# OminiX-ai/OminiX-MLX

Hardware: AMD Instinct MI355X
Metric: decode_tokens_per_sec (higher is better)
Workload: dtype bf16

## Files before the change

include/omx.h:

```cpp
#ifndef OMX_H
#define OMX_H

#include <stddef.h>
#include <stdint.h>

#ifdef __cplusplus
extern "C" {
#endif

typedef enum omx_dtype_ {
    OMX_BOOL = 0, OMX_UINT8 = 1, OMX_UINT16 = 2, OMX_UINT32 = 3, OMX_UINT64 = 4,
    OMX_INT8 = 5, OMX_INT16 = 6, OMX_INT32 = 7, OMX_INT64 = 8,
    OMX_FLOAT16 = 9, OMX_FLOAT32 = 10, OMX_FLOAT64 = 11, OMX_BFLOAT16 = 12, OMX_COMPLEX64 = 13
} omx_dtype;

typedef void* omx_stream;

const char* omx_version(void);
int omx_experiments_built(void);
typedef void (*omx_error_handler_func)(const char* msg, void* data);
void omx_set_error_handler(omx_error_handler_func handler, void* data, void (*dtor)(void*));
const char* omx_last_error(void);
void omx_clear_error(void);
int omx_device_count(int* count);
// ... 119 lines not shown
int omx_qwen3_batch_create_kv(omx_qwen3_batch* out, omx_qwen3 m, int n_slots, int max_context, int kv_bits);
int omx_qwen3_batch_kv_bytes(omx_qwen3_batch b, size_t* bytes);
int omx_qwen3_batch_kv_read(omx_qwen3_batch b, int slot, int layer, int first, int n, void* k_rows, void* v_rows, void* k_scales,
                            void* k_biases, void* v_scales, void* v_biases);
int omx_qwen3_batch_debug_attention(omx_qwen3_batch b, int layer, const int* slots, int n, const void* q, void* out);
int omx_qwen3_batch_destroy(omx_qwen3_batch b);
int omx_qwen3_batch_set_sampler(omx_qwen3_batch b, int slot, float temperature, uint64_t seed);
int omx_qwen3_batch_set_sampling(omx_qwen3_batch b, int slot, const omx_sampling* p, uint64_t seed);
int omx_qwen3_batch_prefill(omx_qwen3_batch b, int slot, const uint32_t* prompt, int n_prompt, uint32_t* first_token);
int omx_qwen3_batch_decode(omx_qwen3_batch b, const int* slots, int n_slots, int n_steps, uint32_t* tokens_out);
int omx_qwen3_batch_logits(omx_qwen3_batch b, int slot, void* host_bf16, int n);
int omx_qwen3_batch_offset(omx_qwen3_batch b, int slot, int* offset);
int omx_qwen3_batch_trim(omx_qwen3_batch b, int slot, int n, uint32_t next_token);
int omx_qwen3_batch_reset(omx_qwen3_batch b, int slot);
int omx_qwen3_batch_fork(omx_qwen3_batch b, int src, int dst, int resample, uint32_t* first_token);
int omx_qwen3_batch_shared(omx_qwen3_batch b, int slot, int* owner, int* shared_len);
int omx_qwen3_batch_last_decode_ms(omx_qwen3_batch b, float* ms);
int omx_bench_qwen3_per_op(omx_qwen3 model, const omx_qwen3_config* cfg, const uint32_t* prompt, int n_prompt, int n_new,
                           uint32_t* tokens_out, double* prefill_ms, double* ms_per_token, double* calls_per_token);
int omx_qwen3_last_decode_ms(omx_qwen3 m, float* ms);
int omx_qwen3_last_prefill_ms(omx_qwen3 m, float* ms);
int omx_qwen3_dequant_bytes(omx_qwen3 m, size_t* bytes);
int omx_qwen3_debug_read(omx_qwen3 m, const char* name, void* host, size_t n_elems);
int omx_debug_gemv(void* out, unsigned long long* argmax_slot, const void* x, const void* norm_w, const void* resid, const void* bias,
                   const void* w0, const void* w1, const void* w2, int n0, int n1, int N, int K, int pro, int epi, int f16, float eps,
                   int single_round, omx_stream stream);
int omx_debug_gemv_grid(int N, int K);
typedef struct omx_gemv_ex_ {
    void* out; unsigned long long* argmax_slot; int argmax_slot_n;
    const void* x; const void* norm_w; const void* resid; const void* bias;
    const void* w0; const void* w1; const void* w2; int n0, n1, N, K, pro, epi, f16; float eps; int single_round;
    int rows_per_wave, row_offset;
    const float* x_partial; int x_partial_n; void* x_out; const void* out_scale;
    int n_batch, x_div; long long x_bstride, out_bstride_bytes; const unsigned* w_sel; long long w_estride; int w_sel_lo, w_sel_n;
    int dry_run;
    int route_nv, route_ksplit, route_tail, route_rows_per_wave, route_blocks;
} omx_gemv_ex;
int omx_debug_gemv_ex(omx_gemv_ex* a, omx_stream stream);
typedef struct omx_qgemv_member_ { const void* w; const void* scales; const void* biases; int n, bits, group; } omx_qgemv_member;
typedef struct omx_qgemv_ex_ {
    omx_qgemv_member m[3];
    int N, K, group, bits, pro, epi; float eps; int single_round;
    int scales_f16, use_sb, use_tiles, mfma, row_offset, rolled_stage;
    int n_batch, x_div; const unsigned* w_sel; long long w_estride, s_estride; int w_sel_lo, w_sel_n, n_experts;
    const void* x; const void* norm_w; const void* resid;
    void* out; float* out_f32; unsigned long long* argmax_slot; int argmax_slot_n;
// ... 226 lines not shown
```

ominix-mlx_amd/csrc/attn.hpp:

```cpp
#pragma once
#include "common.hpp"

namespace omx {

struct AttnDecodeArgs {
    const bf16_t* q;
    const bf16_t* k;
    const bf16_t* v;
    int64_t kv_batch_stride, kv_head_stride;
    int B, H, Hkv, Tk;
    float scale;
    int mask_mode;
    const void* mask;
    int nsplit;
    float* ws_o;
    float* ws_ml;
    bf16_t* out;
    int64_t q_bs, q_hs;
    int causal_tail;
};

struct AttnStepArgs {
    const bf16_t* qkv;
    bf16_t* k;
    bf16_t* v;
    int64_t kv_head_stride;
    int H, Hkv, cap;
    float scale, eps;
    const bf16_t* q_norm_w;
    const bf16_t* k_norm_w;
    const float* rope_cur;
    const int* pos_ptr;
    const unsigned* seq_ptr;
    unsigned tag_mul, tag_add;
    int chunk;
    int nsplit;
    uint64_t* ws;
    bf16_t* out;
    unsigned* abort_flag;
    unsigned long long* trace;
    const bf16_t* o_w;
    const bf16_t* o_resid;
    bf16_t* o_out;
    float* o_out_f32;
// ... 28 lines not shown
```

ominix-mlx_amd/csrc/attn_step.hip:

```cpp
#include <algorithm>

#include "attn.hpp"
#include "act16.hpp"
#include "gemv_parts.hpp"
#include "granule.hpp"
#include "launch_timing.hpp"

namespace omx {

namespace {

constexpr int kBlock = 512;
constexpr int kWaves = 8;
constexpr unsigned kSpinLimit = 1u << 15;

template <int N>
__device__ __forceinline__ float swap_halves(float v) {
    if (N == 16) return dpp_f<0x128>(v);
    return dpp_f<0x1B>(dpp_f<kDppHalfMirror>(v));
}

template <bool F16 = false>
__device__ __forceinline__ void unpack8(const u32x4 r, float (&x)[8]) {
#pragma unroll
// ... 79 lines not shown
}

constexpr int kKU = 3;

template <bool F16>
__device__ __forceinline__ float dot8_16(const u32x4 a, const u32x4 b) {
    if constexpr (!F16) return dot8_bf16(a, b);
    float d = 0.f;
#pragma unroll
    for (int e = 0; e < 4; ++e) d = Act16<true>::dot2(a[e], b[e], d);
    return d;
}

__device__ __forceinline__ float dot8_chain(const u32x4 w, const u32x4 xp, float acc) {
#pragma unroll
    for (int i = 0; i < 4; ++i) {
        acc = fmaf(bf16lo(w[i]), bf16lo(xp[i]), acc);
        acc = fmaf(bf16hi(w[i]), bf16hi(xp[i]), acc);
    }
    return acc;
}

constexpr int kORows = 4;

template <int NVW>
__device__ __forceinline__ void oproj_await_vector(const AttnStepArgs& a, u32x4* sm_x, unsigned tag, int lane, int wave) {
    asm volatile("s_waitcnt vmcnt(0)" ::: "memory");
    if (wave == 0) {
        constexpr int SEGS = NVW * 8;
        const uint64_t* probe = a.xg + (size_t)min(lane, SEGS - 1) * 32 + 31;
        for (unsigned spins = 0; spins < kSpinLimit; ++spins) {
            const unsigned long long g = ld_granule(probe);
            if (__all((unsigned)(g >> 32) == tag)) break;
            __builtin_amdgcn_s_sleep(4);
        }
    }
    __syncthreads();
    constexpr int GP = (NVW + 1) / 2;
    static_assert((NVW * 256) % GP == 0, "a thread takes all of its granules or none");
    bool done = (int)threadIdx.x * GP >= NVW * 256;
    unsigned* sx = reinterpret_cast<unsigned*>(sm_x);
    for (unsigned spins = 0;; ++spins) {
        if (!done) {
            unsigned long long g[GP];
#pragma unroll
            for (int i = 0; i < GP; ++i) g[i] = ld_granule(a.xg + (size_t)threadIdx.x * GP + i);
            bool ok = true;
#pragma unroll
            for (int i = 0; i < GP; ++i) ok &= (unsigned)(g[i] >> 32) == tag;
            if (ok) {
#pragma unroll
                for (int i = 0; i < GP; ++i) sx[threadIdx.x * GP + i] = (unsigned)g[i];
                done = true;
            }
        }
        if (__syncthreads_and(done)) break;
        if (spins >= kSpinLimit) {
            if (threadIdx.x == 0) __hip_atomic_store(a.abort_flag, 1u, __ATOMIC_RELAXED, __HIP_MEMORY_SCOPE_AGENT);
            break;
        }
        __builtin_amdgcn_s_sleep(2);
    }
}

constexpr int kGuPairs = 6, kGuHidden = 4096, kGuNV = kGuHidden / 512;

__device__ __forceinline__ void gateup_issue(const AttnStepArgs& a, u32x4 (*w)[kGuNV], int pair, int lane) {
    const u32x4* g = reinterpret_cast<const u32x4*>(a.gu_gate + (size_t)pair * kGuHidden);
    const u32x4* u = reinterpret_cast<const u32x4*>(a.gu_up + (size_t)pair * kGuHidden);
#pragma unroll
    for (int j = 0; j < kGuNV; ++j) {
        w[0][j] = ld_nt(g + j * 64 + lane);
        w[1][j] = ld_nt(u + j * 64 + lane);
    }
    __builtin_amdgcn_sched_barrier(0);
}

__device__ __forceinline__ void gateup_reduce(const AttnStepArgs& a, const u32x4 (*w)[kGuNV], const u32x4* xs, int pair, int lane) {
    typedef Act16<false> A;
    float acc[2] = {0.f, 0.f};
#pragma unroll
    for (int j = 0; j < kGuNV; ++j) {
        const u32x4 xp = xs[j * 64 + lane];
        float xf[8];
#pragma unroll
        for (int q = 0; q < 4; ++q) {
            xf[2 * q] = A::lo(xp[q]);
            xf[2 * q + 1] = A::hi(xp[q]);
        }
#pragma unroll
        for (int r = 0; r < 2; ++r) acc[r] = dot8(w[r][j], xf, acc[r]);
    }
#pragma unroll
    for (int r = 0; r < 2; ++r) acc[r] = wave_sum(acc[r]);
    if (lane == 0) a.gu_out[pair] = epi_bits<EPI_SWIGLU, A>(acc[0], acc[1], (bf16_t)0, 0);
}

template <bool TRACE>
__device__ __forceinline__ void gateup_phase(const AttnStepArgs& a, u32x4* xs, float* red, const uint16_t* sm_pub, unsigned tag, int lane,
                                             int wave, int pub_row0, int pub_rows, unsigned long long* tr) {
    typedef Act16<false> A;
    const int pair0 = (((int)blockIdx.y * (int)gridDim.x + (int)blockIdx.x) * kWaves + wave) * kGuPairs;
    u32x4 wA[2][kGuNV];
    constexpr int PV = kGuNV * 64 / 256;
    u32x4 nwv[PV];
#pragma unroll
    for (int i = 0; i < PV; ++i) nwv[i] = *(reinterpret_cast<const u32x4*>(a.gu_norm_w) + (threadIdx.x & 255) + i * 256);
    u32x4 wB[2][kGuNV];
    if (wave != 0) gateup_issue(a, wA, pair0, lane);
    lds_barrier();
    if (wave == 0) {
        if (lane < pub_rows / 2) st_granule_u32(a.hg + pub_row0 / 2 + lane, tag, reinterpret_cast<const unsigned*>(sm_pub)[lane]);
        constexpr int GPL = kGuHidden / 2 / 64;
        for (unsigned spins = 0; spins < kSpinLimit; ++spins) {
            const unsigned long long g = ld_granule(a.hg + (size_t)lane * GPL + (GPL - 1));
            if (__all((unsigned)(g >> 32) == tag)) break;
            __builtin_amdgcn_s_sleep(4);
        }
        unsigned long long g[GPL];
        for (unsigned spins = 0;; ++spins) {
#pragma unroll
            for (int i = 0; i < GPL; ++i) g[i] = ld_granule(a.hg + (size_t)i * 64 + lane);
            bool ok = true;
#pragma unroll
            for (int i = 0; i < GPL; ++i) ok &= (unsigned)(g[i] >> 32) == tag;
            if (__all(ok)) break;
            if (spins >= kSpinLimit) {
                if (lane == 0) __hip_atomic_store(a.abort_flag, 1u, __ATOMIC_RELAXED, __HIP_MEMORY_SCOPE_AGENT);
                break;
            }
            __builtin_amdgcn_s_sleep(4);
        }
        unsigned* sx = reinterpret_cast<unsigned*>(xs);
#pragma unroll
        for (int i = 0; i < GPL; ++i) sx[i * 64 + lane] = (unsigned)g[i];
        if (TRACE && lane == 0 && pub_rows > 0) tr[4] = wall_clock64();
        gateup_issue(a, wA, pair0, lane);
    }
    lds_barrier();
    rmsnorm_in_lds<A, PV>(xs, red, nwv, kGuHidden, a.eps, threadIdx.x < 256);
    static_assert(kGuPairs % 2 == 0, "whole double-buffer rounds");
#pragma unroll
    for (int p = 0; p < kGuPairs; p += 2) {
        gateup_issue(a, wB, pair0 + p + 1, lane);
        gateup_reduce(a, wA, xs, pair0 + p, lane);
        if (TRACE && p == 0 && threadIdx.x == 0) tr[7] = wall_clock64();
        if (p + 2 < kGuPairs) gateup_issue(a, wA, pair0 + p + 2, lane);
        gateup_reduce(a, wB, xs, pair0 + p + 1, lane);
    }
}

template <int NVW, int R, bool GU = false>
__device__ __forceinline__ void oproj_phase(const AttnStepArgs& a, u32x4* sm_x, unsigned tag, int lane, int wave, int o_row0,
                                            unsigned long long* tr, uint16_t* sm_pub = nullptr, int pub_row0 = 0) {
    u32x4 ow[R][NVW];
#pragma unroll
    for (int r = 0; r < R; ++r) {
        const int row = min(o_row0 + r, a.o_rows - 1);
        const u32x4* p = reinterpret_cast<const u32x4*>(a.o_w + (size_t)row * (NVW * 512));
#pragma unroll
        for (int j = 0; j < NVW; ++j) ow[r][j] = __builtin_nontemporal_load(p + j * 64 + lane);
    }
    bf16_t o_res[R];
#pragma unroll
    for (int r = 0; r < R; ++r) o_res[r] = a.o_resid[min(o_row0 + r, a.o_rows - 1)];
    __builtin_amdgcn_sched_barrier(0);
    oproj_await_vector<NVW>(a, sm_x, tag, lane, wave);
    if (tr && threadIdx.x == 0) tr[5] = wall_clock64();
    float acc[R];
#pragma unroll
    for (int r = 0; r < R; ++r) acc[r] = 0.f;
// ... 105 lines not shown
            if (o_row0 + r < a.o_rows) a.o_out[o_row0 + r] = f32_to_bf16(bf16_to_f32(o_res[r]) + round_bf16(acc[r]));
    }
    if (tr && threadIdx.x == 0) tr[6] = wall_clock64();
}


template <int D, int GT, bool TRACE, int NVW, bool F16 = false, bool GU = false>
__global__ __launch_bounds__(kBlock, 1) void attn_step_kernel(const AttnStepArgs a) {
    static_assert(!F16 || NVW == 0, "the O projection rides in the launch for bfloat16 models only");
    static_assert(!GU || (NVW == kGuNV && D == 128), "gate/up follows the bf16 O projection of hidden 4096 only");
    typedef Act16<F16> A16;
    constexpr int LPR = D / 8;
    constexpr int TPW = 64 / LPR;
    constexpr bool QO = NVW >= 100;
    constexpr int NV = QO ? NVW - 100 : NVW;
    constexpr bool OPROJ = NV > 0;
    extern __shared__ __attribute__((aligned(16))) unsigned char smem[];
    float* sm_o = reinterpret_cast<float*>(smem);
    float* sm_m = sm_o + kWaves * TPW * GT * D;
    float* sm_l = sm_m + kWaves * GT;
    u32x4* sm_q = reinterpret_cast<u32x4*>(sm_l + kWaves * GT);
    u32x4* sm_x = sm_q + (GT + 1) * LPR;
    float* sm_xsum = reinterpret_cast<float*>(sm_x + NV * 64);

    const int lane = threadIdx.x & 63;
    const int wave = threadIdx.x >> 6;
    const int c = lane % LPR;
    const int sg = lane / LPR;
    const int kvh = blockIdx.x, split = blockIdx.y;
    const int G = a.H / a.Hkv;
    unsigned long long* tr = TRACE ? a.trace + ((size_t)split * a.Hkv + kvh) * 8 : nullptr;
    if (TRACE && threadIdx.x == 0) tr[0] = wall_clock64();

    bf16_t* Kb = a.k + (size_t)kvh * a.kv_head_stride;
    bf16_t* Vb = a.v + (size_t)kvh * a.kv_head_stride;
    const int t_begin = split * a.chunk;
    const int n_units = a.chunk / TPW;

    const bf16_t* kraw = a.qkv + (size_t)a.H * D + (size_t)kvh * D;
    const bool does_q = wave < GT, does_k = wave == GT % kWaves;
    const bf16_t* my_raw = does_q ? a.qkv + (size_t)(kvh * G + min(wave, G - 1)) * D : kraw;
    const u32x4 raw0 = *reinterpret_cast<const u32x4*>(my_raw + c * 8);
    const u32x4 raw1 = *reinterpret_cast<const u32x4*>(kraw + c * 8);
    const u32x4 vnew = *reinterpret_cast<const u32x4*>(kraw + (size_t)a.Hkv * D + c * 8);
    const int i0 = (c % (LPR / 2)) * 8;
    const f32x4* cp = reinterpret_cast<const f32x4*>(a.rope_cur + i0);
    const f32x4* sp = reinterpret_cast<const f32x4*>(a.rope_cur + D / 2 + i0);
    const f32x4 c0 = cp[0], c1 = cp[1], s0 = sp[0], s1 = sp[1];
    u32x4 wq_raw = {0, 0, 0, 0}, wk_raw = {0, 0, 0, 0};
    if (a.q_norm_w) {
        wq_raw = *reinterpret_cast<const u32x4*>(a.q_norm_w + c * 8);
        wk_raw = *reinterpret_cast<const u32x4*>(a.k_norm_w + c * 8);
    }
    u32x4 kr[kKU], vr[kKU];
    auto issue_kv = [&](int u0) {
// ... 149 lines not shown
            }
            uint64_t* gr = a.ws + ((size_t)(kvh * G + g) * a.nsplit + split) * (D + 2);
            st_granule(gr + d, tag, O);
            if (d == 0) {
                st_granule(gr + D, tag, M);
                st_granule(gr + D + 1, tag, L);
            }
        }
    }
    if (TRACE && threadIdx.x == 0) tr[3] = wall_clock64();

    if (OPROJ && split >= G) {
        const int g = ((split - G) * (int)gridDim.x + kvh) * kWaves + wave;
        const bool hi = g < a.o_nhi;
        const int rows = hi ? a.o_rpw : a.o_rpw - 1;
        const int o_row0 = hi ? g * a.o_rpw : a.o_nhi * a.o_rpw + (g - a.o_nhi) * (a.o_rpw - 1);
        unsigned long long* otr = TRACE ? tr : nullptr;
        if constexpr (GU) {
            auto row0_of = [&](int w) { return w < a.o_nhi ? w * a.o_rpw : a.o_nhi * a.o_rpw + (w - a.o_nhi) * (a.o_rpw - 1); };
            const int pub_row0 = row0_of(g - wave), pub_rows = row0_of(g - wave + kWaves) - pub_row0;
            uint16_t* sm_pub = reinterpret_cast<uint16_t*>(sm_l);
            if (rows == 2) oproj_phase<NV, 2, true>(a, sm_x, tag, lane, wave, o_row0, otr, sm_pub, pub_row0);
            else oproj_phase<NV, 3, true>(a, sm_x, tag, lane, wave, o_row0, otr, sm_pub, pub_row0);
            gateup_phase<TRACE>(a, sm_x, sm_m, sm_pub, tag, lane, wave, pub_row0, pub_rows, otr);
            return;
        } else
        if constexpr (QO) {
            if (rows <= 1) oproj_phase_q4<NV, 1>(a, sm_x, sm_xsum, tag, lane, wave, o_row0, otr);
            else if (rows == 2) oproj_phase_q4<NV, 2>(a, sm_x, sm_xsum, tag, lane, wave, o_row0, otr);
            else if (rows == 3) oproj_phase_q4<NV, 3>(a, sm_x, sm_xsum, tag, lane, wave, o_row0, otr);
            else oproj_phase_q4<NV, 4>(a, sm_x, sm_xsum, tag, lane, wave, o_row0, otr);
        } else {
            if (rows <= 1) oproj_phase<(NV > 0 ? NV : 1), 1>(a, sm_x, tag, lane, wave, o_row0, otr);
            else if (rows == 2) oproj_phase<(NV > 0 ? NV : 1), 2>(a, sm_x, tag, lane, wave, o_row0, otr);
            else if (rows == 3) oproj_phase<(NV > 0 ? NV : 1), 3>(a, sm_x, tag, lane, wave, o_row0, otr);
            else oproj_phase<(NV > 0 ? NV : 1), 4>(a, sm_x, tag, lane, wave, o_row0, otr);
        }
        return;
    }

    if (split < G && wave < D / 64) {
        const int head = kvh * G + split;
        const uint64_t* base = a.ws + (size_t)head * a.nsplit * (D + 2);
        bf16_t* out = a.out + (size_t)head * D;
        const int dim = wave * 64 + lane;
        const int nb = (a.nsplit + 15) / 16;
        uint64_t* xg_head = OPROJ ? a.xg + (size_t)head * (D / 2) : nullptr;
        if (nb <= 1) gather_head<D, 1, F16>(a, base, n_active, tag, lane, dim, out, xg_head);
        else if (nb == 2) gather_head<D, 2, F16>(a, base, n_active, tag, lane, dim, out, xg_head);
        else gather_head<D, 3, F16>(a, base, n_active, tag, lane, dim, out, xg_head);
        if (TRACE && threadIdx.x == 0) tr[4] = wall_clock64();
    }
    if constexpr (GU) {
        lds_barrier();
        gateup_phase<TRACE>(a, sm_x, sm_m, nullptr, tag, lane, wave, 0, 0, TRACE ? tr : nullptr);
    }
}

}

int attn_step_block_tokens(int D) { return 64 / (D / 8); }

constexpr int kMaxSplits = 48;
void attn_step_plan(int tk_max, int Hkv, int G, int D, int* chunk, int* nsplit) {
    const int unit = attn_step_block_tokens(D);
    int target = std::max(1, std::min(kMaxSplits, 256 / std::max(Hkv, 1)));
    if (const char* v = getenv("OMX_ATTN_STEP_SPLITS")) target = std::max(1, std::min(kMaxSplits, atoi(v)));
    int ch = unit * ((tk_max + unit * target - 1) / (unit * target));
    if (ch < unit) ch = unit;
    int ns = (tk_max + ch - 1) / ch;
    if (ns < G) ns = G;
    *chunk = ch;
    *nsplit = ns;
}

size_t attn_step_ws_granules(int H, int D) { return (size_t)H * kMaxSplits * (D + 2); }

static int oproj_rows_per_wave(int H, int Hkv, int nsplit, int o_rows) {
    const int waves = (Hkv * nsplit - H) * kWaves;
    return waves > 0 ? (o_rows + waves - 1) / waves : 1 << 20;
}
bool attn_step_oproj_ok(int H, int Hkv, int D, int nsplit, int o_rows) {
    const int K = H * D, nvw = K / 512;
    return K % 512 == 0 && (nvw == 1 || nvw == 2 || nvw == 4 || nvw == 7 || nvw == 8) && oproj_rows_per_wave(H, Hkv, nsplit, o_rows) <= kORows;
}

bool attn_step_oproj_q4_ok(int H, int Hkv, int D, int nsplit, int o_rows, int group) {
    const int K = H * D;
    return (K == 2048 || K == 4096) && (group == 32 || group == 64 || group == 128) && attn_step_oproj_ok(H, Hkv, D, nsplit, o_rows);
}

bool attn_step_gateup_ok(int H, int Hkv, int D, int nsplit, int o_rows, int gu_rows) {
    const int blocks = Hkv * nsplit, waves = (blocks - H) * kWaves;
    if (D != 128 || H * D != kGuHidden || o_rows != kGuHidden || H / std::max(Hkv, 1) != 4 || blocks != 256) return false;
    if (gu_rows != blocks * kWaves * kGuPairs || !attn_step_oproj_ok(H, Hkv, D, nsplit, o_rows)) return false;
    return oproj_rows_per_wave(H, Hkv, nsplit, o_rows) == 3 && (o_rows - waves * 2) % kWaves == 0;
}

int launch_attn_step(const AttnStepArgs& a_in, int D, hipStream_t s) {
    AttnStepArgs a = a_in;
    const int G = a.H / a.Hkv;
    OMX_REQUIRE(a.H % a.Hkv == 0 && G >= 1 && G <= 8, "decode attention: %d query heads over %d KV heads unsupported (group of at most 8)", a.H, a.Hkv);
    OMX_REQUIRE(a.nsplit >= G && a.nsplit <= kMaxSplits && a.chunk > 0 && a.chunk % attn_step_block_tokens(D) == 0 && a.Hkv * a.nsplit <= 256,
                "decode attention: bad split plan (chunk %d, %d splits, group %d, %d kv heads)", a.chunk, a.nsplit, G, a.Hkv);
    OMX_REQUIRE(a.ws && a.rope_cur && a.pos_ptr && a.seq_ptr && a.abort_flag && a.tag_mul > a.tag_add - 1u && a.tag_add >= 1u,
                "decode attention: missing step state");
    int nvw = 0;
    const bool qo = a.o_wq != nullptr;
    if (qo)
        OMX_REQUIRE(!a.o_w && a.o_sb && a.o_out && !a.o_out_f32 && attn_step_oproj_q4_ok(a.H, a.Hkv, D, a.nsplit, a.o_rows, a.o_group),
                    "decode attention + packed O projection: shape does not qualify (H*D = %d, group %d)", a.H * D, a.o_group);
    if (a.o_w || qo) {
        OMX_REQUIRE(a.o_resid && (a.o_out || a.o_out_f32) && a.xg && attn_step_oproj_ok(a.H, a.Hkv, D, a.nsplit, a.o_rows),
                    "decode attention + O projection: shape does not qualify (H*D = %d, %d rows, %d blocks)", a.H * D, a.o_rows, a.Hkv * a.nsplit);
        nvw = a.H * D / 512;
        a.o_rpw = oproj_rows_per_wave(a.H, a.Hkv, a.nsplit, a.o_rows);
        const int waves = (a.Hkv * a.nsplit - a.H) * kWaves;
        a.o_nhi = a.o_rpw > 1 ? a.o_rows - waves * (a.o_rpw - 1) : waves;
// ... 4 lines not shown
                    "decode attention + gate/up: shape does not qualify (%d blocks, %d O rows, %d pairs)", a.Hkv * a.nsplit, a.o_rows, a.gu_rows);
    const dim3 grid(a.Hkv, a.nsplit), block(kBlock);
    const int gt = G <= 1 ? 1 : G <= 2 ? 2 : G <= 4 ? 4 : 8;
#define OMX_ATTN_LAUNCH(DD, GG, TT, NN)                                                                                  \
    {                                                                                                                    \
        if (shmem > 48 * 1024)                                                                                           \
            OMX_HIP_CHECK(hipFuncSetAttribute((const void*)attn_step_kernel<DD, GG, TT, NN>,                            \
                                              hipFuncAttributeMaxDynamicSharedMemorySize, (int)shmem));                  \
        OMX_LAUNCH_TIMED((attn_step_kernel<DD, GG, TT, NN>), grid, block, shmem, s, a);                                  \
        OMX_LAUNCH_CHECK();                                                                                              \
        return 0;                                                                                                        \
    }
#define OMX_ATTN_LAUNCH_GU(TT)                                                                                           \
    {                                                                                                                    \
        OMX_HIP_CHECK(hipFuncSetAttribute((const void*)attn_step_kernel<128, 4, TT, kGuNV, false, true>,                 \
                                          hipFuncAttributeMaxDynamicSharedMemorySize, (int)shmem));                      \
        OMX_LAUNCH_TIMED((attn_step_kernel<128, 4, TT, kGuNV, false, true>), grid, block, shmem, s, a);                  \
        OMX_LAUNCH_CHECK();                                                                                              \
        return 0;                                                                                                        \
    }
#define OMX_ATTN_STEP_CASE(DD, GG)                                                                                       \
    if (D == DD && gt == GG) {                                                                                           \
        const size_t shmem = ((size_t)kWaves * (64 / (DD / 8)) * GG * DD + 2 * kWaves * GG) * sizeof(float) +            \
                             (size_t)(GG + 1) * (DD / 8) * 16 + (size_t)nvw * 64 * 16 + (qo ? (size_t)nvw * 64 : 0);     \
        if (a.gu_gate) {                            \
            if constexpr (DD == 128 && GG == 4) {                                                                        \
                if (a.trace) OMX_ATTN_LAUNCH_GU(true)                                                                    \
                OMX_ATTN_LAUNCH_GU(false)                                                                                \
            }                                                                                                            \
            return set_error("decode attention + gate/up: no instantiation for head_dim %d, group %d", DD, GG);         \
        }                                                                                                                \
        if (a.trace && !qo) {                           \
            if (nvw == 0) OMX_ATTN_LAUNCH(DD, GG, true, 0)                                                               \
            if (nvw == 8) OMX_ATTN_LAUNCH(DD, GG, true, 8)                                                               \
            return set_error("decode attention: no traced instantiation for H*D = %d", a.H * DD);                       \
        }                                                                                                                \
        if (qo) {                                                                                                        \
            if (nvw == 4) OMX_ATTN_LAUNCH(DD, GG, false, 104)                                                            \
            OMX_ATTN_LAUNCH(DD, GG, false, 108)                                                                          \
        }                                                                                                                \
        if (a.f16) {    \
            if constexpr (DD == 128) {                                                                                   \
                if (nvw == 0) {                                                                                          \
                    if (shmem > 48 * 1024)                                                                               \
                        OMX_HIP_CHECK(hipFuncSetAttribute((const void*)attn_step_kernel<DD, GG, false, 0, true>,        \
                                                          hipFuncAttributeMaxDynamicSharedMemorySize, (int)shmem));      \
                    OMX_LAUNCH_TIMED((attn_step_kernel<DD, GG, false, 0, true>), grid, block, shmem, s, a);              \
// ... 23 lines not shown
```

ominix-mlx_amd/csrc/engine.hip:

```cpp
#include "engine_model.hpp"

namespace omx {
namespace {

__global__ void rope_table_kernel(float* cos_t, float* sin_t, int cap, int half, double neg_log_base_over_half,
                                  double scale) {
    const int idx = blockIdx.x * blockDim.x + threadIdx.x;
    if (idx >= cap * half) return;
    const int t = idx / half, i = idx % half;
    const double ang = ((double)t * scale) * exp((double)i * neg_log_base_over_half);
    double s, c;
    sincos(ang, &s, &c);
    cos_t[idx] = (float)c;
    sin_t[idx] = (float)s;
}


}
}

extern "C" {

int omx_qwen3_create(omx_qwen3* out, const omx_qwen3_config* cfg) {
    OMX_REQUIRE(out && cfg, "omx_qwen3_create: null argument");
// ... 425 lines not shown
            OMX_HIP_CHECK(hipStreamSynchronize(m->stream));
            OMX_HIP_CHECK(hipEventElapsedTime(&m->last_decode_ms, m->ev0, m->ev1));
        }
        unsigned gave_up = 0;
        if (step_gave_up(m, &gave_up)) return 1;
        if (!gave_up) break;
        if (step_fallback(m, st)) return step_health(m);
        if (prepare_step(m, st.pos)) return 1;
    }
    std::vector<uint32_t> ring(m->ring_cap);
    OMX_HIP_CHECK(hipMemcpy(ring.data(), m->out_ring, (size_t)m->ring_cap * 4, hipMemcpyDeviceToHost));
    for (int i = 0; i < n; ++i) tokens_out[i] = ring[(st.out_count + i) % m->ring_cap];
    return 0;
}

int omx_qwen3_last_logits(omx_qwen3 m, void* host_bf16, int n) {
    OMX_REQUIRE(m && host_bf16, "omx_qwen3_last_logits: null argument");
    OMX_REQUIRE(n == m->V, "omx_qwen3_last_logits: expected %d entries, got %d", m->V, n);
    OMX_HIP_CHECK(hipMemcpyAsync(host_bf16, m->logits, (size_t)n * 2, hipMemcpyDeviceToHost, m->stream));
    OMX_HIP_CHECK(hipStreamSynchronize(m->stream));
    return 0;
}

int omx_qwen3_debug_read(omx_qwen3 m, const char* name, void* host, size_t n_elems) {
    OMX_REQUIRE(m && name && host, "omx_qwen3_debug_read: null argument");
    const void* src = nullptr;
    const std::string s(name);
    if (s == "h") src = m->h;
    else if (s == "h2") src = m->h2;
    else if (s == "qkv") src = m->qkv;
    else if (s == "attn_out") src = m->attn_out;
    else if (s == "act") src = m->act;
    else if (s.rfind("g_", 0) == 0 && m->se_gran) {
        const size_t hd = m->cfg.hidden_size, D = m->cfg.head_dim;
        const uint64_t* g = m->se_gran;
        if (s == "g_x") src = g;
        else if (s == "g_x1") src = g + hd / 2;
        else if (s == "g_qkv") src = g + hd;
        else if (s == "g_attn") src = g + hd + (size_t)(m->H + 2 * m->Hkv) * D / 2;
        else if (s == "g_act") src = g + hd + (size_t)(m->H + 2 * m->Hkv) * D / 2 + (size_t)m->H * D / 2;
    }
    else if (s.size() > 1 && (s[0] == 'k' || s[0] == 'v')) {
        const int l = atoi(s.c_str() + 1);
        OMX_REQUIRE(l >= 0 && l < (int)m->kcache.size(), "omx_qwen3_debug_read: bad layer in %s", name);
        src = s[0] == 'k' ? m->kcache[l] : m->vcache[l];
    }
    OMX_REQUIRE(src != nullptr, "omx_qwen3_debug_read: unknown buffer %s", name);
    OMX_HIP_CHECK(hipMemcpyAsync(host, src, n_elems * 2, hipMemcpyDeviceToHost, m->stream));
    OMX_HIP_CHECK(hipStreamSynchronize(m->stream));
    return 0;
}

int omx_qwen3_last_decode_ms(omx_qwen3 m, float* ms) {
    OMX_REQUIRE(m && ms, "omx_qwen3_last_decode_ms: null argument");
    *ms = m->last_decode_ms;
    return 0;
}

int omx_qwen3_stream(omx_qwen3 m, omx_stream* s) {
    OMX_REQUIRE(m && s, "omx_qwen3_stream: null argument");
    *s = (omx_stream)m->stream;
    return 0;
}

int omx_qwen3_debug_trace_step(omx_qwen3 m, unsigned long long* host, size_t n_words, int* blocks) {
    OMX_REQUIRE(m && host && blocks, "omx_qwen3_debug_trace_step: null argument");
    StepState st;
    if (read_step_state(m, &st)) return 1;
    if (prepare_step(m, st.pos)) return 1;
    const size_t per_layer = (size_t)m->attn_nsplit * m->Hkv * 8, need = per_layer * m->cfg.num_hidden_layers;
    OMX_REQUIRE(n_words >= need, "omx_qwen3_debug_trace_step: buffer of %zu words, need %zu", n_words, need);
    unsigned long long* dev = nullptr;
    OMX_HIP_CHECK(hipMalloc(&dev, need * 8));
    OMX_HIP_CHECK(hipMemsetAsync(dev, 0, need * 8, m->stream));
    m->attn_trace = dev;
    const int rc = enqueue_step(m, true);
    m->attn_trace = nullptr;
    if (!rc) {
        OMX_HIP_CHECK(hipStreamSynchronize(m->stream));
        OMX_HIP_CHECK(hipMemcpy(host, dev, need * 8, hipMemcpyDeviceToHost));
    }
    (void)hipFree(dev);
    *blocks = m->attn_nsplit * m->Hkv;
    return rc ? 1 : step_health(m);
}

int omx_qwen3_time_step_kernels(omx_qwen3 m, int steps, float* us) {
    OMX_REQUIRE(m && us && steps > 0, "omx_qwen3_time_step_kernels: bad arguments");
    OMX_REQUIRE(!m->cfg.quant_bits && m->cfg.num_experts == 0 && m->allreduce == nullptr, "omx_qwen3_time_step_kernels: dense bf16 single-rank models only");
    const int L = m->cfg.num_hidden_layers;
    std::vector<hipEvent_t> ev((size_t)(L * kLayerClasses + 2) * 2);
    for (auto& e : ev) OMX_HIP_CHECK(hipEventCreate(&e));
    double sum[KC_COUNT] = {};
// ... 108 lines not shown
```

ominix-mlx_amd/csrc/engine_step.hip:

```cpp
#include "engine_model.hpp"

namespace omx {
namespace {

__device__ __forceinline__ void step_begin(const StepState* st, unsigned* seq, float* rope_cur, const float* rope_cos,
                                           const float* rope_sin, int half) {
    if (blockIdx.x != 0) return;
    if (seq && threadIdx.x == 0) *seq += 1u;
    if (rope_cur && (int)threadIdx.x < 2 * half) {
        const int t = threadIdx.x, pos = st->pos;
        rope_cur[t] = t < half ? rope_cos[(size_t)pos * half + t] : rope_sin[(size_t)pos * half + t - half];
    }
}

template <int BITS>
__global__ __launch_bounds__(256) void qembed_kernel(bf16_t* __restrict__ h, const uint32_t* __restrict__ w,
                                                     const bf16_t* __restrict__ scales, const bf16_t* __restrict__ biases,
                                                     const StepState* st, int hidden, int group, unsigned* seq, float* rope_cur,
                                                     const float* rope_cos, const float* rope_sin, int half, bool scales_f16) {
    constexpr int EPW = 32 / BITS;
    step_begin(st, seq, rope_cur, rope_cos, rope_sin, half);
    const size_t row = st->cur_token;
    const int words = hidden / EPW;
    for (int i = blockIdx.x * blockDim.x + threadIdx.x; i < words; i += gridDim.x * blockDim.x) {
// ... 210 lines not shown
}

static int enqueue_attention(omx_qwen3 m, int l, hipStream_t s, const bf16_t* resid = nullptr, bf16_t* out = nullptr, float* out_f32 = nullptr,
                             bool gateup = false) {
    const omx_qwen3_config& c = m->cfg;
    const int D = c.head_dim;
    const LayerW& L = m->layers[l];
    AttnStepArgs a = {};
    a.qkv = m->qkv;
    a.k = m->kcache[l]; a.v = m->vcache[l];
    a.kv_head_stride = (int64_t)m->cap * D;
    a.H = m->H; a.Hkv = m->Hkv; a.cap = m->cap;
    a.scale = 1.0f / sqrtf((float)D);
    a.eps = c.rms_norm_eps;
    a.q_norm_w = L.q_norm; a.k_norm_w = L.k_norm;
    a.rope_cur = m->rope_cur;
    a.pos_ptr = &m->st->pos;
    a.seq_ptr = m->step_seq;
    a.tag_mul = (unsigned)c.num_hidden_layers; a.tag_add = (unsigned)l + 1u;
    a.chunk = m->attn_chunk; a.nsplit = m->attn_nsplit;
    a.ws = m->attn_gran;
    a.out = m->attn_out;
    a.abort_flag = m->wait_abort;
    a.trace = m->attn_trace ? m->attn_trace + (size_t)l * m->attn_nsplit * m->Hkv * 8 : nullptr;
    a.f16 = m->f16;
    if (resid && (out || out_f32)) {
        a.o_resid = resid; a.o_out = out; a.o_out_f32 = out_f32; a.o_rows = c.hidden_size; a.xg = m->attn_xg;
        if (c.quant_bits) {
            const QMat& o = m->qlayers[l].o;
            a.o_wq = o.w; a.o_sb = o.sb; a.o_group = o.group;
        } else {
            a.o_w = L.o;
        }
    }
    if (gateup) {
        a.gu_gate = L.gate; a.gu_up = L.up; a.gu_norm_w = L.post_ln; a.gu_out = m->act; a.gu_rows = m->I;
        a.hg = m->gateup_gran;
    }
    return launch_attn_step(a, D, s);
}

int enqueue_step_tail(omx_qwen3 m, bool with_head, const bf16_t* h, const float* pending, int pending_n, bool tp) {
    const omx_qwen3_config& c = m->cfg;
    hipStream_t s = m->stream;
    if (!with_head) {
        OMX_LAUNCH(feed_prompt_kernel, 1, 1, 0, s, m->st, m->prompt_dev);
        OMX_LAUNCH_CHECK();
// ... 486 lines not shown
```

ominix-mlx_amd/engine.py:

```python
from __future__ import annotations

import ctypes
import sys
from typing import Dict, Iterator, Optional

import numpy as np

from . import OmxError, Sampling, check, lib, require_device
from .ops import Tensor

c_int, c_float, c_void_p, c_uint32 = ctypes.c_int, ctypes.c_float, ctypes.c_void_p, ctypes.c_uint32


class Qwen3Config(ctypes.Structure):
    _fields_ = [("hidden_size", c_int), ("num_hidden_layers", c_int), ("intermediate_size", c_int),
                ("num_attention_heads", c_int), ("num_key_value_heads", c_int), ("head_dim", c_int),
                ("vocab_size", c_int), ("rms_norm_eps", c_float), ("rope_theta", c_float), ("rope_scale", c_float),
                ("tie_word_embeddings", c_int), ("max_context", c_int), ("tp_rank", c_int), ("tp_size", c_int),
                ("quant_bits", c_int), ("quant_group", c_int), ("num_experts", c_int), ("num_experts_per_tok", c_int),
                ("moe_intermediate_size", c_int), ("moe_mode", c_int), ("norm_topk_prob", c_int), ("no_qk_norm", c_int),
                ("ep_rank", c_int), ("ep_size", c_int), ("attention_bias", c_int), ("quant_scales_f16", c_int),
                ("float16_weights", c_int)]


# ... 52 lines not shown

ENGINE_SIGNATURES = {
    "omx_fill_uniform_2d": (c_int, [c_void_p, ctypes.c_int64, ctypes.c_int64, ctypes.c_int64, ctypes.c_int64,
                                    ctypes.c_int64, c_uint32, c_float, c_float, c_int, c_void_p]),
    "omx_qwen3_create": (c_int, [ctypes.POINTER(c_void_p), ctypes.POINTER(Qwen3Config)]),
    "omx_qwen3_destroy": (c_int, [c_void_p]),
    "omx_qwen3_set_weight": (c_int, [c_void_p, ctypes.c_char_p, c_void_p, ctypes.c_size_t]),
    "omx_qwen3_synth_weights": (c_int, [c_void_p, c_uint32]),
    "omx_qwen3_synth_weights_peaked": (c_int, [c_void_p, c_uint32]),
    "omx_qwen3_set_comm": (c_int, [c_void_p, c_void_p, c_void_p]),
    "omx_qwen3_set_sampler": (c_int, [c_void_p, ctypes.c_float, ctypes.c_uint64]),
    "omx_qwen3_set_sampling": (c_int, [c_void_p, ctypes.POINTER(Sampling), ctypes.c_uint64]),
    "omx_qwen3_sampler_state": (c_int, [c_void_p, c_void_p, c_int]),
    "omx_qwen3_encode": (c_int, [c_void_p, ctypes.POINTER(c_uint32), c_int, c_void_p, ctypes.POINTER(c_int), c_int, c_void_p]),
    "omx_qwen3_reset": (c_int, [c_void_p]),
    "omx_qwen3_offset": (c_int, [c_void_p, ctypes.POINTER(c_int)]),
    "omx_qwen3_prefill": (c_int, [c_void_p, ctypes.POINTER(c_uint32), c_int, ctypes.POINTER(c_uint32)]),
    "omx_qwen3_decode": (c_int, [c_void_p, c_int, ctypes.POINTER(c_uint32)]),
    "omx_qwen3_last_logits": (c_int, [c_void_p, c_void_p, c_int]),
    "omx_qwen3_last_decode_ms": (c_int, [c_void_p, ctypes.POINTER(c_float)]),
    "omx_qwen3_last_prefill_ms": (c_int, [c_void_p, ctypes.POINTER(c_float)]),
    "omx_qwen3_dequant_bytes": (c_int, [c_void_p, ctypes.POINTER(ctypes.c_size_t)]),
    "omx_qwen3_debug_read": (c_int, [c_void_p, ctypes.c_char_p, c_void_p, ctypes.c_size_t]),
    "omx_qwen3_stream": (c_int, [c_void_p, ctypes.POINTER(c_void_p)]),
    "omx_qwen3_step_bytes": (c_int, [c_void_p, c_int, ctypes.POINTER(ctypes.c_double)]),
    "omx_qwen3_decode_path": (c_int, [c_void_p, ctypes.POINTER(c_int)]),
    "omx_qwen3_debug_trace_step": (c_int, [c_void_p, c_void_p, ctypes.c_size_t, ctypes.POINTER(c_int)]),
    "omx_qwen3_time_step_kernels": (c_int, [c_void_p, c_int, ctypes.POINTER(ctypes.c_float)]),
    "omx_qwen3_debug_trace_engine": (c_int, [c_void_p, c_void_p, ctypes.c_size_t, ctypes.POINTER(c_int)]),
    "omx_qwen3_debug_step_forms": (c_int, [c_void_p, ctypes.POINTER(c_int)]),
    "omx_qwen3_debug_raise_give_up": (c_int, [c_void_p]),
    "omx_qwen3_verify": (c_int, [c_void_p, ctypes.POINTER(c_uint32), c_int, ctypes.POINTER(c_uint32)]),
    "omx_qwen3_verify_logits": (c_int, [c_void_p, c_int, c_void_p, c_int]),
    "omx_qwen3_trim": (c_int, [c_void_p, c_int, c_uint32]),
    "omx_qwen3_score": (c_int, [c_void_p, ctypes.POINTER(c_uint32), c_int, ctypes.POINTER(c_uint32), ctypes.POINTER(c_float), ctypes.POINTER(c_uint32)]),
    "omx_qwen3_last_score_ms": (c_int, [c_void_p, ctypes.POINTER(c_float), ctypes.POINTER(c_float)]),
    "omx_qwen3_get_weight": (c_int, [c_void_p, ctypes.c_char_p, ctypes.POINTER(c_void_p), ctypes.POINTER(ctypes.c_size_t)]),
    "omx_qwen3_set_quant_format": (c_int, [c_void_p, ctypes.c_char_p, c_int, c_int]),
    "omx_qwen3_quant_format": (c_int, [c_void_p, ctypes.c_char_p, ctypes.POINTER(c_int), ctypes.POINTER(c_int)]),
    "omx_qwen3_batch_create": (c_int, [ctypes.POINTER(c_void_p), c_void_p, c_int, c_int]),
    "omx_qwen3_batch_destroy": (c_int, [c_void_p]),
    "omx_qwen3_batch_set_sampler": (c_int, [c_void_p, c_int, ctypes.c_float, ctypes.c_uint64]),
    "omx_qwen3_batch_set_sampling": (c_int, [c_void_p, c_int, ctypes.POINTER(Sampling), ctypes.c_uint64]),
    "omx_qwen3_batch_prefill": (c_int, [c_void_p, c_int, ctypes.POINTER(c_uint32), c_int, ctypes.POINTER(c_uint32)]),
    "omx_qwen3_batch_decode": (c_int, [c_void_p, ctypes.POINTER(c_int), c_int, c_int, ctypes.POINTER(c_uint32)]),
    "omx_qwen3_batch_logits": (c_int, [c_void_p, c_int, c_void_p, c_int]),
# ... 549 lines not shown
```

Before: 344.2.

## Balance gate/up pairs across waves with an LDS ticket counter

Replaces the fixed six (gate, up) row pairs per wave with a per-block pool of 48 pairs that waves claim dynamically through an LDS atomic ticket, so waves that finish attention or o-proj early take more rows. Wave 0 now issues its first pair's weight loads before checking the hidden-vector granule tags, which hides the tag read behind those loads. It also widens the trace buffer and adds a debug write API. The cost is an LDS atomic and a readfirstlane per claimed pair, plus a loop whose trip count is no longer fixed at compile time.

```diff
diff --git a/include/omx.h b/include/omx.h
--- a/include/omx.h
+++ b/include/omx.h
@@ -165,6 +165,7 @@
 int omx_qwen3_last_prefill_ms(omx_qwen3 m, float* ms);
 int omx_qwen3_dequant_bytes(omx_qwen3 m, size_t* bytes);
 int omx_qwen3_debug_read(omx_qwen3 m, const char* name, void* host, size_t n_elems);
+int omx_qwen3_debug_write(omx_qwen3 m, const char* name, const void* host, size_t n_elems);
 int omx_debug_gemv(void* out, unsigned long long* argmax_slot, const void* x, const void* norm_w, const void* resid, const void* bias,
                    const void* w0, const void* w1, const void* w2, int n0, int n1, int N, int K, int pro, int epi, int f16, float eps,
                    int single_round, omx_stream stream);
diff --git a/ominix-mlx_amd/csrc/attn.hpp b/ominix-mlx_amd/csrc/attn.hpp
--- a/ominix-mlx_amd/csrc/attn.hpp
+++ b/ominix-mlx_amd/csrc/attn.hpp
@@ -20,6 +20,7 @@
     int causal_tail;
 };
 
+constexpr int kAttnTraceWords = 16;
 struct AttnStepArgs {
     const bf16_t* qkv;
     bf16_t* k;
diff --git a/ominix-mlx_amd/csrc/attn_step.hip b/ominix-mlx_amd/csrc/attn_step.hip
--- a/ominix-mlx_amd/csrc/attn_step.hip
+++ b/ominix-mlx_amd/csrc/attn_step.hip
@@ -125,6 +125,26 @@
 }
 
 constexpr int kORows = 4;
+
+constexpr int kGuBlockPairs = 48, kGuHidden = 4096, kGuNV = kGuHidden / 512;
+enum { kGuTicket = 0, kGuReduced = 1, kGuWords = 4 };
+
+__device__ __forceinline__ int gateup_claim(int* sm_gu, int lane) {
+    int t = 0;
+    if (lane == 0) t = __hip_atomic_fetch_add(sm_gu + kGuTicket, 1, __ATOMIC_RELAXED, __HIP_MEMORY_SCOPE_WORKGROUP);
+    return __builtin_amdgcn_readfirstlane(t);
+}
+
+__device__ __forceinline__ void gateup_issue(const AttnStepArgs& a, u32x4 (*w)[kGuNV], int pair, int lane) {
+    const u32x4* g = reinterpret_cast<const u32x4*>(a.gu_gate + (size_t)pair * kGuHidden);
+    const u32x4* u = reinterpret_cast<const u32x4*>(a.gu_up + (size_t)pair * kGuHidden);
+#pragma unroll
+    for (int j = 0; j < kGuNV; ++j) {
+        w[0][j] = ld_nt(g + j * 64 + lane);
+        w[1][j] = ld_nt(u + j * 64 + lane);
+    }
+    __builtin_amdgcn_sched_barrier(0);
+}
 
 template <int NVW>
 __device__ __forceinline__ void oproj_await_vector(const AttnStepArgs& a, u32x4* sm_x, unsigned tag, int lane, int wave) {
@@ -166,19 +186,6 @@
     }
 }
 
-constexpr int kGuPairs = 6, kGuHidden = 4096, kGuNV = kGuHidden / 512;
-
-__device__ __forceinline__ void gateup_issue(const AttnStepArgs& a, u32x4 (*w)[kGuNV], int pair, int lane) {
-    const u32x4* g = reinterpret_cast<const u32x4*>(a.gu_gate + (size_t)pair * kGuHidden);
-    const u32x4* u = reinterpret_cast<const u32x4*>(a.gu_up + (size_t)pair * kGuHidden);
-#pragma unroll
-    for (int j = 0; j < kGuNV; ++j) {
-        w[0][j] = ld_nt(g + j * 64 + lane);
-        w[1][j] = ld_nt(u + j * 64 + lane);
-    }
-    __builtin_amdgcn_sched_barrier(0);
-}
-
 __device__ __forceinline__ void gateup_reduce(const AttnStepArgs& a, const u32x4 (*w)[kGuNV], const u32x4* xs, int pair, int lane) {
     typedef Act16<false> A;
     float acc[2] = {0.f, 0.f};
@@ -200,17 +207,20 @@
 }
 
 template <bool TRACE>
-__device__ __forceinline__ void gateup_phase(const AttnStepArgs& a, u32x4* xs, float* red, const uint16_t* sm_pub, unsigned tag, int lane,
-                                             int wave, int pub_row0, int pub_rows, unsigned long long* tr) {
+__device__ __forceinline__ void gateup_phase(const AttnStepArgs& a, u32x4* xs, float* red, int* sm_gu, const uint16_t* sm_pub, unsigned tag,
+                                             int lane, int wave, int pub_row0, int pub_rows, unsigned long long* tr) {
     typedef Act16<false> A;
-    const int pair0 = (((int)blockIdx.y * (int)gridDim.x + (int)blockIdx.x) * kWaves + wave) * kGuPairs;
-    u32x4 wA[2][kGuNV];
+    const int pair0 = ((int)blockIdx.y * (int)gridDim.x + (int)blockIdx.x) * kGuBlockPairs;
     constexpr int PV = kGuNV * 64 / 256;
     u32x4 nwv[PV];
 #pragma unroll
     for (int i = 0; i < PV; ++i) nwv[i] = *(reinterpret_cast<const u32x4*>(a.gu_norm_w) + (threadIdx.x & 255) + i * 256);
-    u32x4 wB[2][kGuNV];
-    if (wave != 0) gateup_issue(a, wA, pair0, lane);
+    u32x4 wA[2][kGuNV], wB[2][kGuNV];
+    int tA = 0, tB;
+    if (wave != 0) {
+        tA = gateup_claim(sm_gu, lane);
+        gateup_issue(a, wA, pair0 + tA, lane);
+    }
     lds_barrier();
     if (wave == 0) {
         if (lane < pub_rows / 2) st_granule_u32(a.hg + pub_row0 / 2 + lane, tag, reinterpret_cast<const unsigned*>(sm_pub)[lane]);
@@ -221,35 +231,83 @@
             __builtin_amdgcn_s_sleep(4);
         }
         unsigned long long g[GPL];
-        for (unsigned spins = 0;; ++spins) {
-#pragma unroll
-            for (int i = 0; i < GPL; ++i) g[i] = ld_granule(a.hg + (size_t)i * 64 + lane);
-            bool ok = true;
-#pragma unroll
-            for (int i = 0; i < GPL; ++i) ok &= (unsigned)(g[i] >> 32) == tag;
-            if (__all(ok)) break;
-            if (spins >= kSpinLimit) {
-                if (lane == 0) __hip_atomic_store(a.abort_flag, 1u, __ATOMIC_RELAXED, __HIP_MEMORY_SCOPE_AGENT);
-                break;
-            }
-            __builtin_amdgcn_s_sleep(4);
+#pragma unroll
+        for (int i = 0; i < GPL; ++i) g[i] = ld_granule(a.hg + (size_t)i * 64 + lane);
+        __builtin_amdgcn_sched_barrier(0);
+        lds_barrier();
+        tA = gateup_claim(sm_gu, lane);
+        gateup_issue(a, wA, pair0 + tA, lane);
+        unsigned bad = 0;
+#pragma unroll
+        for (int i = 0; i < GPL; ++i) bad |= (unsigned)(g[i] >> 32) ^ tag;
+        asm volatile("; hidden row: tags read behind the first (gate, up) pair" : "+v"(bad));
+        if (!__all(bad == 0)) {
+            for (unsigned spins = 0;; ++spins) {
+#pragma unroll
+                for (int i = 0; i < GPL; ++i) g[i] = ld_granule(a.hg + (size_t)i * 64 + lane);
+                bool ok = true;
+#pragma unroll
+                for (int i = 0; i < GPL; ++i) ok &= (unsigned)(g[i] >> 32) == tag;
+                if (__all(ok)) break;
+                if (spins >= kSpinLimit) {
+                    if (lane == 0) __hip_atomic_store(a.abort_flag, 1u, __ATOMIC_RELAXED, __HIP_MEMORY_SCOPE_AGENT);
+                    break;
+                }
+                __builtin_amdgcn_s_sleep(4);
+            }
         }
         unsigned* sx = reinterpret_cast<unsigned*>(xs);
 #pragma unroll
         for (int i = 0; i < GPL; ++i) sx[i * 64 + lane] = (unsigned)g[i];
         if (TRACE && lane == 0 && pub_rows > 0) tr[4] = wall_clock64();
-        gateup_issue(a, wA, pair0, lane);
+        tB = gateup_claim(sm_gu, lane);
+    } else {
+        lds_barrier();
+        tB = gateup_claim(sm_gu, lane);
+        gateup_issue(a, wB, pair0 + tB, lane);
     }
     lds_barrier();
     rmsnorm_in_lds<A, PV>(xs, red, nwv, kGuHidden, a.eps, threadIdx.x < 256);
-    static_assert(kGuPairs % 2 == 0, "whole double-buffer rounds");
-#pragma unroll
-    for (int p = 0; p < kGuPairs; p += 2) {
-        gateup_issue(a, wB, pair0 + p + 1, lane);
-        gateup_reduce(a, wA, xs, pair0 + p, lane);
-        if (TRACE && p == 0 && threadIdx.x == 0) tr[7] = wall_clock64();
-        if (p + 2 < kGuPairs) gateup_issue(a, wA, pair0 + p + 2, lane);
-        gateup_reduce(a, wB, xs, pair0 + p + 1, lane);
+    if (wave == 0) {
+        gateup_issue(a, wB, pair0 + tB, lane);
+        gateup_reduce(a, wA, xs, pair0 + tA, lane);
+        if (TRACE && threadIdx.x == 0) tr[7] = wall_clock64();
+        asm volatile("; first pair reduced: wave 0, its second pair just asked for" ::: "memory");
+    } else {
+        gateup_reduce(a, wA, xs, pair0 + tA, lane);
+        asm volatile("; first pair reduced: the second pair came in through the hop" ::: "memory");
+    }
+    int n_reduced = 1;
+    int nA = gateup_claim(sm_gu, lane), nB;
+    for (;;) {
+        if (nA >= kGuBlockPairs) {
+            gateup_reduce(a, wB, xs, pair0 + tB, lane);
+            ++n_reduced;
+            break;
+        }
+        tA = nA;
+        gateup_issue(a, wA, pair0 + tA, lane);
+        nB = gateup_claim(sm_gu, lane);
+        gateup_reduce(a, wB, xs, pair0 + tB, lane);
+        if (nB >= kGuBlockPairs) {
+            gateup_reduce(a, wA, xs, pair0 + tA, lane);
+            n_reduced += 2;
+            break;
+        }
+        tB = nB;
+        gateup_issue(a, wB, pair0 + tB, lane);
+        nA = gateup_claim(sm_gu, lane);
+        gateup_reduce(a, wA, xs, pair0 + tA, lane);
+        n_reduced += 2;
+    }
+    if constexpr (TRACE) {
+        if (lane == 0) {
+            __hip_atomic_fetch_add(sm_gu + kGuReduced, n_reduced, __ATOMIC_RELAXED, __HIP_MEMORY_SCOPE_WORKGROUP);
+            if (wave == 0) tr[8] = wall_clock64();
+            if (wave == kWaves - 1) tr[9] = wall_clock64();
+        }
+        lds_barrier();
+        if (threadIdx.x == 0) tr[10] = (unsigned long long)sm_gu[kGuReduced];
     }
 }
 
@@ -401,6 +459,7 @@
     u32x4* sm_q = reinterpret_cast<u32x4*>(sm_l + kWaves * GT);
     u32x4* sm_x = sm_q + (GT + 1) * LPR;
     float* sm_xsum = reinterpret_cast<float*>(sm_x + NV * 64);
+    int* sm_gu = reinterpret_cast<int*>(sm_x + NV * 64);
 
     const int lane = threadIdx.x & 63;
     const int wave = threadIdx.x >> 6;
@@ -408,8 +467,11 @@
     const int sg = lane / LPR;
     const int kvh = blockIdx.x, split = blockIdx.y;
     const int G = a.H / a.Hkv;
-    unsigned long long* tr = TRACE ? a.trace + ((size_t)split * a.Hkv + kvh) * 8 : nullptr;
+    unsigned long long* tr = TRACE ? a.trace + ((size_t)split * a.Hkv + kvh) * kAttnTraceWords : nullptr;
     if (TRACE && threadIdx.x == 0) tr[0] = wall_clock64();
+    if constexpr (GU) {
+        if (threadIdx.x < kGuWords) sm_gu[threadIdx.x] = 0;
+    }
 
     bf16_t* Kb = a.k + (size_t)kvh * a.kv_head_stride;
     bf16_t* Vb = a.v + (size_t)kvh * a.kv_head_stride;
@@ -605,7 +667,7 @@
             uint16_t* sm_pub = reinterpret_cast<uint16_t*>(sm_l);
             if (rows == 2) oproj_phase<NV, 2, true>(a, sm_x, tag, lane, wave, o_row0, otr, sm_pub, pub_row0);
             else oproj_phase<NV, 3, true>(a, sm_x, tag, lane, wave, o_row0, otr, sm_pub, pub_row0);
-            gateup_phase<TRACE>(a, sm_x, sm_m, sm_pub, tag, lane, wave, pub_row0, pub_rows, otr);
+            gateup_phase<TRACE>(a, sm_x, sm_m, sm_gu, sm_pub, tag, lane, wave, pub_row0, pub_rows, otr);
             return;
         } else
         if constexpr (QO) {
@@ -636,7 +698,7 @@
     }
     if constexpr (GU) {
         lds_barrier();
-        gateup_phase<TRACE>(a, sm_x, sm_m, nullptr, tag, lane, wave, 0, 0, TRACE ? tr : nullptr);
+        gateup_phase<TRACE>(a, sm_x, sm_m, sm_gu, nullptr, tag, lane, wave, 0, 0, TRACE ? tr : nullptr);
     }
 }
 
@@ -676,7 +738,7 @@
 bool attn_step_gateup_ok(int H, int Hkv, int D, int nsplit, int o_rows, int gu_rows) {
     const int blocks = Hkv * nsplit, waves = (blocks - H) * kWaves;
     if (D != 128 || H * D != kGuHidden || o_rows != kGuHidden || H / std::max(Hkv, 1) != 4 || blocks != 256) return false;
-    if (gu_rows != blocks * kWaves * kGuPairs || !attn_step_oproj_ok(H, Hkv, D, nsplit, o_rows)) return false;
+    if (gu_rows != blocks * kGuBlockPairs || !attn_step_oproj_ok(H, Hkv, D, nsplit, o_rows)) return false;
     return oproj_rows_per_wave(H, Hkv, nsplit, o_rows) == 3 && (o_rows - waves * 2) % kWaves == 0;
 }
 
@@ -727,7 +789,8 @@
 #define OMX_ATTN_STEP_CASE(DD, GG)                                                                                       \
     if (D == DD && gt == GG) {                                                                                           \
         const size_t shmem = ((size_t)kWaves * (64 / (DD / 8)) * GG * DD + 2 * kWaves * GG) * sizeof(float) +            \
-                             (size_t)(GG + 1) * (DD / 8) * 16 + (size_t)nvw * 64 * 16 + (qo ? (size_t)nvw * 64 : 0);     \
+                             (size_t)(GG + 1) * (DD / 8) * 16 + (size_t)nvw * 64 * 16 + (qo ? (size_t)nvw * 64 : 0) +    \
+                             (a.gu_gate ? kGuWords * sizeof(int) : 0);                                                   \
         if (a.gu_gate) {                            \
             if constexpr (DD == 128 && GG == 4) {                                                                        \
                 if (a.trace) OMX_ATTN_LAUNCH_GU(true)                                                                    \
diff --git a/ominix-mlx_amd/csrc/engine.hip b/ominix-mlx_amd/csrc/engine.hip
--- a/ominix-mlx_amd/csrc/engine.hip
+++ b/ominix-mlx_amd/csrc/engine.hip
@@ -471,9 +471,8 @@
     return 0;
 }
 
-int omx_qwen3_debug_read(omx_qwen3 m, const char* name, void* host, size_t n_elems) {
-    OMX_REQUIRE(m && name && host, "omx_qwen3_debug_read: null argument");
-    const void* src = nullptr;
+static void* debug_buffer(omx_qwen3 m, const char* name) {
+    void* src = nullptr;
     const std::string s(name);
     if (s == "h") src = m->h;
     else if (s == "h2") src = m->h2;
@@ -482,7 +481,7 @@
     else if (s == "act") src = m->act;
     else if (s.rfind("g_", 0) == 0 && m->se_gran) {
         const size_t hd = m->cfg.hidden_size, D = m->cfg.head_dim;
-        const uint64_t* g = m->se_gran;
+        uint64_t* g = m->se_gran;
         if (s == "g_x") src = g;
         else if (s == "g_x1") src = g + hd / 2;
         else if (s == "g_qkv") src = g + hd;
@@ -491,11 +490,25 @@
     }
     else if (s.size() > 1 && (s[0] == 'k' || s[0] == 'v')) {
         const int l = atoi(s.c_str() + 1);
-        OMX_REQUIRE(l >= 0 && l < (int)m->kcache.size(), "omx_qwen3_debug_read: bad layer in %s", name);
-        src = s[0] == 'k' ? m->kcache[l] : m->vcache[l];
-    }
-    OMX_REQUIRE(src != nullptr, "omx_qwen3_debug_read: unknown buffer %s", name);
+        if (l >= 0 && l < (int)m->kcache.size()) src = s[0] == 'k' ? m->kcache[l] : m->vcache[l];
+    }
+    return src;
+}
+
+int omx_qwen3_debug_read(omx_qwen3 m, const char* name, void* host, size_t n_elems) {
+    OMX_REQUIRE(m && name && host, "omx_qwen3_debug_read: null argument");
+    const void* src = debug_buffer(m, name);
+    OMX_REQUIRE(src != nullptr, "omx_qwen3_debug_read: unknown buffer or layer %s", name);
     OMX_HIP_CHECK(hipMemcpyAsync(host, src, n_elems * 2, hipMemcpyDeviceToHost, m->stream));
+    OMX_HIP_CHECK(hipStreamSynchronize(m->stream));
+    return 0;
+}
+
+int omx_qwen3_debug_write(omx_qwen3 m, const char* name, const void* host, size_t n_elems) {
+    OMX_REQUIRE(m && name && host, "omx_qwen3_debug_write: null argument");
+    void* dst = debug_buffer(m, name);
+    OMX_REQUIRE(dst != nullptr, "omx_qwen3_debug_write: unknown buffer %s", name);
+    OMX_HIP_CHECK(hipMemcpyAsync(dst, host, n_elems * 2, hipMemcpyHostToDevice, m->stream));
     OMX_HIP_CHECK(hipStreamSynchronize(m->stream));
     return 0;
 }
@@ -517,7 +530,7 @@
     StepState st;
     if (read_step_state(m, &st)) return 1;
     if (prepare_step(m, st.pos)) return 1;
-    const size_t per_layer = (size_t)m->attn_nsplit * m->Hkv * 8, need = per_layer * m->cfg.num_hidden_layers;
+    const size_t per_layer = (size_t)m->attn_nsplit * m->Hkv * kAttnTraceWords, need = per_layer * m->cfg.num_hidden_layers;
     OMX_REQUIRE(n_words >= need, "omx_qwen3_debug_trace_step: buffer of %zu words, need %zu", n_words, need);
     unsigned long long* dev = nullptr;
     OMX_HIP_CHECK(hipMalloc(&dev, need * 8));
diff --git a/ominix-mlx_amd/csrc/engine_step.hip b/ominix-mlx_amd/csrc/engine_step.hip
--- a/ominix-mlx_amd/csrc/engine_step.hip
+++ b/ominix-mlx_amd/csrc/engine_step.hip
@@ -256,7 +256,7 @@
     a.ws = m->attn_gran;
     a.out = m->attn_out;
     a.abort_flag = m->wait_abort;
-    a.trace = m->attn_trace ? m->attn_trace + (size_t)l * m->attn_nsplit * m->Hkv * 8 : nullptr;
+    a.trace = m->attn_trace ? m->attn_trace + (size_t)l * m->attn_nsplit * m->Hkv * kAttnTraceWords : nullptr;
     a.f16 = m->f16;
     if (resid && (out || out_f32)) {
         a.o_resid = resid; a.o_out = out; a.o_out_f32 = out_f32; a.o_rows = c.hidden_size; a.xg = m->attn_xg;
diff --git a/ominix-mlx_amd/engine.py b/ominix-mlx_amd/engine.py
--- a/ominix-mlx_amd/engine.py
+++ b/ominix-mlx_amd/engine.py
@@ -98,6 +98,7 @@
     "omx_qwen3_last_prefill_ms": (c_int, [c_void_p, ctypes.POINTER(c_float)]),
     "omx_qwen3_dequant_bytes": (c_int, [c_void_p, ctypes.POINTER(ctypes.c_size_t)]),
     "omx_qwen3_debug_read": (c_int, [c_void_p, ctypes.c_char_p, c_void_p, ctypes.c_size_t]),
+    "omx_qwen3_debug_write": (c_int, [c_void_p, ctypes.c_char_p, c_void_p, ctypes.c_size_t]),
     "omx_qwen3_stream": (c_int, [c_void_p, ctypes.POINTER(c_void_p)]),
     "omx_qwen3_step_bytes": (c_int, [c_void_p, c_int, ctypes.POINTER(ctypes.c_double)]),
     "omx_qwen3_decode_path": (c_int, [c_void_p, ctypes.POINTER(c_int)]),
```

New measurement: 348.4, median of 6. +1.2%, better.
